# HengyiWang/MorpheuS

Hardware: AMD Instinct MI355X
Metric: rays/sec (fwd+bwd, 128 samples/ray) (higher is better)
Workload: dtype f32 (exact 3 x bf16 operand split on the bf16 MFMA pipe, fp32 accumulate)

## Files before the change

### morpheus_amd/csrc/mlp_b3.hip

```cpp
#include "mlp_dev.h"
#include <stdlib.h>

#define B3_THREADS 512
#define B3_BLOCK_PTS 256
#define B3_L0_F4 2560
#define B3_LH_F4 6144
#define B3_KH_F4 3072
#define B3_L5_F4 1536
#define B3_NET_F4 (B3_L0_F4 + 4 * B3_LH_F4 + B3_L5_F4)
#define B3_LDS_BYTES (B3_LH_F4 * 16 + 1024)

extern __shared__ f32x4 lds_b3[];
constexpr int B3_Q4_FILL = 6;
#define B3_PARK_STORES_EIGHTH 8
#define B3_PARK_STORES_HALF (4 * B3_PARK_STORES_EIGHTH)
#define B3_KEEP_BWD B3_PARK_STORES_HALF
static_assert(B3_KEEP_BWD <= B3_PARK_STORES_HALF && B3_PARK_STORES_HALF <= 63, "vmcnt(KEEP) must not exceed the stores behind the DMA");

#ifdef MH_PHASE_TRACE
__device__ long long mh_b3_trace[256 * 64];
#define B3_TRACE_ON (((threadIdx.x & 255) == 0) && (blockIdx.x % 64 == 0) && (blockIdx.x / 64 < 128))
#define B3_TRACE_ROW ((blockIdx.x / 64) * 2 + (threadIdx.x >> 8))
#define B3_STAMP(slot)                                                                          \
    do {                                                                                        \
        if (B3_TRACE_ON) mh_b3_trace[B3_TRACE_ROW * 64 + (slot)] = (long long)__builtin_amdgcn_s_memtime(); \
    } while (0)
#define B3_STAMP_REAL(slot)                                                                     \
    do {                                                                                        \
        if (B3_TRACE_ON) mh_b3_trace[B3_TRACE_ROW * 64 + (slot)] = (long long)__builtin_amdgcn_s_memrealtime(); \
    } while (0)
extern "C" int mh_b3_trace_read(long long *dst_host) {
    return hipMemcpyFromSymbol(dst_host, HIP_SYMBOL(mh_b3_trace), sizeof(long long) * 256 * 64) == hipSuccess ? 0 : 2;
}
#else
#define B3_STAMP(slot) do { } while (0)
#define B3_STAMP_REAL(slot) do { } while (0)
#endif

template <int N_F4, int NTHR = B3_THREADS>
__device__ __forceinline__ void b3_stage_issue(const f32x4 *__restrict__ src) {
    static_assert(N_F4 % NTHR == 0, "whole rounds of the block");
    const int wave = threadIdx.x >> 6;
#pragma unroll
    for (int k = 0; k < N_F4 / NTHR; k++)
        __builtin_amdgcn_global_load_lds((const __attribute__((address_space(1))) void *)(src + k * NTHR + threadIdx.x),
                                         (__attribute__((address_space(3))) void *)(lds_b3 + k * NTHR + wave * 64), 16, 0, 0);
}
__device__ __forceinline__ void b3_stage_wait() {
    asm volatile("s_waitcnt vmcnt(0)" ::: "memory");
    __syncthreads();
}
template <int YOUNGER>
__device__ __forceinline__ void b3_stage_wait_keep() {
    static_assert(YOUNGER >= 0 && YOUNGER <= 63, "vmcnt is a 6-bit field");
    asm volatile("s_waitcnt vmcnt(%0)" ::"n"(YOUNGER) : "memory");
    __syncthreads();
}
__device__ __forceinline__ void b3_dma_fence() { asm volatile("" ::: "memory"); }

template <int KS, int MT, bool ZERO = false>
__device__ __forceinline__ void b3_layer(const f32x4 *__restrict__ w, const Frag (&bh)[8], const Frag (&bm)[8], const Frag (&bl)[8],
                                         f32x16 (&acc)[MT], int lane) {
    constexpr int PL = MT * KS * 64;
    constexpr int NT = MT >= 2 ? 2 : 1;
    const f32x16 zero = {0.f, 0.f, 0.f, 0.f, 0.f, 0.f, 0.f, 0.f, 0.f, 0.f, 0.f, 0.f, 0.f, 0.f, 0.f, 0.f};
#pragma unroll
    for (int s = 0; s < KS; s++) {
#pragma unroll
        for (int mp = 0; mp < MT; mp += NT) {
            Frag ah[NT], am[NT], al[NT];
#pragma unroll
            for (int t = 0; t < NT; t++) {
                ah[t].f = w[0 * PL + ((mp + t) * KS + s) * 64 + lane];
                am[t].f = w[1 * PL + ((mp + t) * KS + s) * 64 + lane];
                al[t].f = w[2 * PL + ((mp + t) * KS + s) * 64 + lane];
            }
#pragma unroll
            for (int t = 0; t < NT; t++)
                acc[mp + t] = __builtin_amdgcn_mfma_f32_32x32x16_bf16(al[t].h, bh[s].h, (ZERO && s == 0) ? zero : acc[mp + t], 0, 0, 0);
#pragma unroll
            for (int t = 0; t < NT; t++) acc[mp + t] = __builtin_amdgcn_mfma_f32_32x32x16_bf16(am[t].h, bm[s].h, acc[mp + t], 0, 0, 0);
#pragma unroll
            for (int t = 0; t < NT; t++) acc[mp + t] = __builtin_amdgcn_mfma_f32_32x32x16_bf16(ah[t].h, bl[s].h, acc[mp + t], 0, 0, 0);
#pragma unroll
            for (int t = 0; t < NT; t++) acc[mp + t] = __builtin_amdgcn_mfma_f32_32x32x16_bf16(am[t].h, bh[s].h, acc[mp + t], 0, 0, 0);
#pragma unroll
            for (int t = 0; t < NT; t++) acc[mp + t] = __builtin_amdgcn_mfma_f32_32x32x16_bf16(ah[t].h, bm[s].h, acc[mp + t], 0, 0, 0);
#pragma unroll
            for (int t = 0; t < NT; t++) acc[mp + t] = __builtin_amdgcn_mfma_f32_32x32x16_bf16(ah[t].h, bh[s].h, acc[mp + t], 0, 0, 0);
        }
    }
}

__device__ __forceinline__ void mfma_results_settle() {
    __builtin_amdgcn_sched_barrier(0);
    asm volatile("s_nop 15");
    __builtin_amdgcn_sched_barrier(0);
}

template <int T0, int S0>
__device__ __forceinline__ void b3_quarter(const f32x4 *__restrict__ w, const Frag (&bh)[8], const Frag (&bm)[8], const Frag (&bl)[8],
                                           f32x16 (&acc)[4], int lane) {
    constexpr int PLH = 4 * 4 * 64;
#pragma unroll
    for (int s = S0; s < S0 + 4; s++) {
        Frag ah[2], am[2], al[2];
        const f32x4 *wk = w + (S0 / 4) * B3_KH_F4 + ((s & 3)) * 64 + lane;
#pragma unroll
        for (int t = 0; t < 2; t++) {
            ah[t].f = wk[0 * PLH + (T0 + t) * 256];
            am[t].f = wk[1 * PLH + (T0 + t) * 256];
            al[t].f = wk[2 * PLH + (T0 + t) * 256];
        }
#pragma unroll
        for (int t = 0; t < 2; t++) acc[T0 + t] = __builtin_amdgcn_mfma_f32_32x32x16_bf16(al[t].h, bh[s].h, acc[T0 + t], 0, 0, 0);
#pragma unroll
        for (int t = 0; t < 2; t++) acc[T0 + t] = __builtin_amdgcn_mfma_f32_32x32x16_bf16(am[t].h, bm[s].h, acc[T0 + t], 0, 0, 0);
#pragma unroll
        for (int t = 0; t < 2; t++) acc[T0 + t] = __builtin_amdgcn_mfma_f32_32x32x16_bf16(ah[t].h, bl[s].h, acc[T0 + t], 0, 0, 0);
#pragma unroll
        for (int t = 0; t < 2; t++) acc[T0 + t] = __builtin_amdgcn_mfma_f32_32x32x16_bf16(am[t].h, bh[s].h, acc[T0 + t], 0, 0, 0);
#pragma unroll
        for (int t = 0; t < 2; t++) acc[T0 + t] = __builtin_amdgcn_mfma_f32_32x32x16_bf16(ah[t].h, bm[s].h, acc[T0 + t], 0, 0, 0);
#pragma unroll
        for (int t = 0; t < 2; t++) acc[T0 + t] = __builtin_amdgcn_mfma_f32_32x32x16_bf16(ah[t].h, bh[s].h, acc[T0 + t], 0, 0, 0);
    }
}

template <int T0>
__device__ __forceinline__ void b3_quarter_step(const f32x4 *__restrict__ w, const Frag (&bh)[8], const Frag (&bm)[8],
                                                const Frag (&bl)[8], f32x16 (&acc)[4], int lane, int s) {
    constexpr int PLH = 4 * 4 * 64;
    Frag ah[2], am[2], al[2];
    const f32x4 *wk = w + (s >> 2) * B3_KH_F4 + (s & 3) * 64 + lane;
#pragma unroll
    for (int t = 0; t < 2; t++) {
        ah[t].f = wk[0 * PLH + (T0 + t) * 256];
        am[t].f = wk[1 * PLH + (T0 + t) * 256];
        al[t].f = wk[2 * PLH + (T0 + t) * 256];
    }
#pragma unroll
    for (int t = 0; t < 2; t++) acc[T0 + t] = __builtin_amdgcn_mfma_f32_32x32x16_bf16(al[t].h, bh[s].h, acc[T0 + t], 0, 0, 0);
#pragma unroll
    for (int t = 0; t < 2; t++) acc[T0 + t] = __builtin_amdgcn_mfma_f32_32x32x16_bf16(am[t].h, bm[s].h, acc[T0 + t], 0, 0, 0);
#pragma unroll
    for (int t = 0; t < 2; t++) acc[T0 + t] = __builtin_amdgcn_mfma_f32_32x32x16_bf16(ah[t].h, bl[s].h, acc[T0 + t], 0, 0, 0);
#pragma unroll
    for (int t = 0; t < 2; t++) acc[T0 + t] = __builtin_amdgcn_mfma_f32_32x32x16_bf16(am[t].h, bh[s].h, acc[T0 + t], 0, 0, 0);
#pragma unroll
    for (int t = 0; t < 2; t++) acc[T0 + t] = __builtin_amdgcn_mfma_f32_32x32x16_bf16(ah[t].h, bm[s].h, acc[T0 + t], 0, 0, 0);
#pragma unroll
    for (int t = 0; t < 2; t++) acc[T0 + t] = __builtin_amdgcn_mfma_f32_32x32x16_bf16(ah[t].h, bh[s].h, acc[T0 + t], 0, 0, 0);
}

template <bool PARK>
__device__ __forceinline__ void b3_epilogue_eighth(f32x16 (&acc)[4], float *__restrict__ ht, uint32_t (&mt)[4], int pt, int h,
                                                   Frag (&bh)[8], Frag (&bm)[8], Frag (&bl)[8], int t, int s2) {
#pragma unroll
    for (int r = 8 * s2; r < 8 * s2 + 8; r++) acc[t][r] = relu_i(acc[t][r]);
    if (PARK) {
#pragma unroll
        for (int r = 8 * s2; r < 8 * s2 + B3_PARK_STORES_EIGHTH; r++) PARK_STORE(acc[t][r], &ht[(32 * t + acc_row(r, h)) * TILE + pt]);
    }
    uint32_t m = 0;
#pragma unroll
    for (int r = 8 * s2 + 7; r >= 8 * s2; r--) m = push_nz(m, acc[t][r]);
    mt[t] |= m << (8 * s2);
#pragma unroll
    for (int e2 = 0; e2 < 4; e2++)
        split2(acc[t][8 * s2 + 2 * e2], acc[t][8 * s2 + 2 * e2 + 1], bh[2 * t + s2].u[e2], bm[2 * t + s2].u[e2], bl[2 * t + s2].u[e2]);
}

template <int T0, bool PARK>
__device__ __forceinline__ void b3_epilogue_half(f32x16 (&acc)[4], float *__restrict__ ht, uint32_t (&mt)[4], int pt, int h,
                                                 Frag (&bh)[8], Frag (&bm)[8], Frag (&bl)[8]) {
#pragma unroll
    for (int t = T0; t < T0 + 2; t++) {
#pragma unroll
        for (int r = 0; r < 16; r++) acc[t][r] = relu_i(acc[t][r]);
        if (PARK) {
#pragma unroll
            for (int r = 0; r < 16; r++) PARK_STORE(acc[t][r], &ht[(32 * t + acc_row(r, h)) * TILE + pt]);
        }
        uint32_t m = 0;
#pragma unroll
        for (int r = 15; r >= 0; r--) m = push_nz(m, acc[t][r]);
        mt[t] = m;
#pragma unroll
        for (int s2 = 0; s2 < 2; s2++)
#pragma unroll
            for (int e2 = 0; e2 < 4; e2++)
                split2(acc[t][8 * s2 + 2 * e2], acc[t][8 * s2 + 2 * e2 + 1], bh[2 * t + s2].u[e2], bm[2 * t + s2].u[e2],
                       bl[2 * t + s2].u[e2]);
    }
}

#define B3_SLOT_F4 B3_KH_F4
#define B3_BIASROW_F4 (2 * B3_SLOT_F4)
constexpr int B3_Q_FILL = 6;

template <int N_F4, int NTHR>
__device__ __forceinline__ void b3_slot_issue(const f32x4 *__restrict__ base, int off_f4, int slot) {
    static_assert(N_F4 % NTHR == 0, "whole rounds of the block");
    asm volatile("" : "+s"(off_f4));
    const f32x4 *src = base + off_f4 + threadIdx.x;
    f32x4 *dst = lds_b3 + slot * B3_SLOT_F4 + (threadIdx.x >> 6) * 64;
#pragma unroll
    for (int k = 0; k < N_F4 / NTHR; k++)
        __builtin_amdgcn_global_load_lds((const __attribute__((address_space(1))) void *)(src + k * NTHR),
                                         (__attribute__((address_space(3))) void *)(dst + k * NTHR), 16, 0, 0);
}
__device__ __forceinline__ void b3_bias_issue(const float *__restrict__ bias, int off_floats, int n_f4, int row) {
    asm volatile("" : "+s"(off_floats));
    if ((int)threadIdx.x < n_f4)
        __builtin_amdgcn_global_load_lds((const __attribute__((address_space(1))) void *)(reinterpret_cast<const f32x4 *>(bias + off_floats) + threadIdx.x),
                                         (__attribute__((address_space(3))) void *)(lds_b3 + B3_BIASROW_F4 + row * 32), 16, 0, 0);
}
template <int T0, int NT, int MT>
__device__ __forceinline__ void b3_acc_bias_row(f32x16 (&acc)[MT], int h, int row) {
    const f32x4 *b = lds_b3 + B3_BIASROW_F4 + row * 32;
#pragma unroll
    for (int t = T0; t < T0 + NT; t++)
#pragma unroll
        for (int r4 = 0; r4 < 4; r4++) {
            const f32x4 v = b[8 * t + 2 * r4 + h];
#pragma unroll
            for (int c = 0; c < 4; c++) acc[t][4 * r4 + c] = v[c];
        }
}
template <int KEEP>
__device__ __forceinline__ void b3_point() {
    static_assert(KEEP >= 0 && KEEP <= 63, "vmcnt is a 6-bit field");
    asm volatile("s_waitcnt vmcnt(%0) lgkmcnt(0)" ::"n"(KEEP) : "memory");
    __builtin_amdgcn_s_barrier();
    asm volatile("" ::: "memory");
}
template <int T0>
__device__ __forceinline__ void b3_step(const f32x4 *__restrict__ wk, const Frag (&bh)[8], const Frag (&bm)[8], const Frag (&bl)[8],
                                        f32x16 (&acc)[4], int lane, int s) {
    constexpr int PLH = 4 * 4 * 64;
    Frag ah[2], am[2], al[2];
    const f32x4 *w = wk + (s & 3) * 64 + lane;
#pragma unroll
    for (int t = 0; t < 2; t++) {
        ah[t].f = w[0 * PLH + (T0 + t) * 256];
        am[t].f = w[1 * PLH + (T0 + t) * 256];
        al[t].f = w[2 * PLH + (T0 + t) * 256];
    }
#pragma unroll
    for (int t = 0; t < 2; t++) acc[T0 + t] = __builtin_amdgcn_mfma_f32_32x32x16_bf16(al[t].h, bh[s].h, acc[T0 + t], 0, 0, 0);
#pragma unroll
    for (int t = 0; t < 2; t++) acc[T0 + t] = __builtin_amdgcn_mfma_f32_32x32x16_bf16(am[t].h, bm[s].h, acc[T0 + t], 0, 0, 0);
#pragma unroll
    for (int t = 0; t < 2; t++) acc[T0 + t] = __builtin_amdgcn_mfma_f32_32x32x16_bf16(ah[t].h, bl[s].h, acc[T0 + t], 0, 0, 0);
#pragma unroll
    for (int t = 0; t < 2; t++) acc[T0 + t] = __builtin_amdgcn_mfma_f32_32x32x16_bf16(am[t].h, bh[s].h, acc[T0 + t], 0, 0, 0);
#pragma unroll
    for (int t = 0; t < 2; t++) acc[T0 + t] = __builtin_amdgcn_mfma_f32_32x32x16_bf16(ah[t].h, bm[s].h, acc[T0 + t], 0, 0, 0);
#pragma unroll
    for (int t = 0; t < 2; t++) acc[T0 + t] = __builtin_amdgcn_mfma_f32_32x32x16_bf16(ah[t].h, bh[s].h, acc[T0 + t], 0, 0, 0);
}
__device__ __forceinline__ void b3_l5_step(const f32x4 *__restrict__ w, const Frag (&bh)[8], const Frag (&bm)[8], const Frag (&bl)[8],
                                           f32x16 &o, int lane, int s) {
    Frag ah, am, al;
    ah.f = w[0 * 512 + s * 64 + lane];
    am.f = w[1 * 512 + s * 64 + lane];
    al.f = w[2 * 512 + s * 64 + lane];
    o = __builtin_amdgcn_mfma_f32_32x32x16_bf16(al.h, bh[s].h, o, 0, 0, 0);
    o = __builtin_amdgcn_mfma_f32_32x32x16_bf16(am.h, bm[s].h, o, 0, 0, 0);
    o = __builtin_amdgcn_mfma_f32_32x32x16_bf16(ah.h, bl[s].h, o, 0, 0, 0);
    o = __builtin_amdgcn_mfma_f32_32x32x16_bf16(am.h, bh[s].h, o, 0, 0, 0);
    o = __builtin_amdgcn_mfma_f32_32x32x16_bf16(ah.h, bm[s].h, o, 0, 0, 0);
    o = __builtin_amdgcn_mfma_f32_32x32x16_bf16(ah.h, bh[s].h, o, 0, 0, 0);
}
template <int S0>
__device__ __forceinline__ void b3_pin_slices(Frag (&bh)[8], Frag (&bm)[8], Frag (&bl)[8]) {
#pragma unroll
    for (int s = S0; s < S0 + 4; s++)
        asm volatile("" : "+v"(bh[s].u[0]), "+v"(bh[s].u[1]), "+v"(bh[s].u[2]), "+v"(bh[s].u[3]), "+v"(bm[s].u[0]), "+v"(bm[s].u[1]),
                     "+v"(bm[s].u[2]), "+v"(bm[s].u[3]), "+v"(bl[s].u[0]), "+v"(bl[s].u[1]), "+v"(bl[s].u[2]), "+v"(bl[s].u[3]));
}
template <int N, int FILL>
__device__ __forceinline__ void b3_interleave() {
#pragma unroll
    for (int g = 0; g < N; g++) {
        __builtin_amdgcn_sched_group_barrier(0x008, 1, 0);
        __builtin_amdgcn_sched_group_barrier(0x002, FILL, 0);
    }
}

__device__ __forceinline__ uint32_t b3_or_half(uint32_t v) {
    v |= (uint32_t)__builtin_amdgcn_update_dpp(0, (int)v, 0x111, 0xf, 0xf, false);
    v |= (uint32_t)__builtin_amdgcn_update_dpp(0, (int)v, 0x112, 0xf, 0xf, false);
    v |= (uint32_t)__builtin_amdgcn_update_dpp(0, (int)v, 0x114, 0xf, 0xf, false);
    v |= (uint32_t)__builtin_amdgcn_update_dpp(0, (int)v, 0x118, 0xf, 0xf, false);
    v |= (uint32_t)__builtin_amdgcn_update_dpp(0, (int)v, 0x142, 0xa, 0xf, false);
    return v;
}
__device__ __forceinline__ void b3_park_line_word(float *__restrict__ tile, int idx, int pt, int h, uint32_t lo, uint32_t hi) {
    lo = b3_or_half(lo);
    hi = b3_or_half(hi);
    if (pt == 31) reinterpret_cast<uint2 *>(tile + WARP_LINE_ROW * TILE)[idx * 2 + h] = make_uint2(lo, hi);
}

template <int NW, bool PARK>
// ... 30 lines not shown

    for (int net = 0; net < 2; net++) {
        const f32x4 *wn = net ? w3_t : w3_d;
        const float *bs = net ? bias_t : bias_d;
        const float *b0 = (net ? bias0_t : bias0_d) + (int64_t)sl * 128;
        float *ht = PARK ? tile + (64 + net * 640) * TILE : nullptr;
        f32x16 acc[4];
        Frag bh[8], bm[8], bl[8];
        uint32_t mt[4] = {0u, 0u, 0u, 0u};
#pragma unroll
        for (int s = 0; s < 3; s++)
#pragma unroll
            for (int e2 = 0; e2 < 4; e2++) split2(bin0[8 * s + 2 * e2], bin0[8 * s + 2 * e2 + 1], bh[s].u[e2], bm[s].u[e2], bl[s].u[e2]);
        acc_bias<4>(acc, b0, h);
        b3_point<0>();
        b3_layer<3, 4>(slot0, bh, bm, bl, acc, lane);
        b3_point<0>();
        b3_slot_issue<B3_KH_F4, NT>(wn, B3_L0_F4 + B3_KH_F4, 0);
        b3_dma_fence();
        b3_epilogue_half<0, PARK>(acc, ht, mt, pt, h, bh, bm, bl);
        __builtin_amdgcn_sched_barrier(0);
        for (int l = 1; l <= 4; l++) {
            const int row = l & 1;
            float *hp = ht + (l - 1) * 128 * TILE, *hl = ht + l * 128 * TILE;
            if (net == 0) B3_STAMP((l - 1) * 8 + 0);
            if (net == 0 && l == 1) B3_STAMP_REAL(62);
            b3_acc_bias_row<0, 2, 4>(acc, h, row);
            mt[2] = mt[3] = 0u;
#pragma unroll
            for (int c = 0; c < 4; c++) {
                b3_step<0>(slot1, bh, bm, bl, acc, lane, c);
                b3_epilogue_eighth<PARK>(acc, hp, mt, pt, h, bh, bm, bl, 2 + (c >> 1), c & 1);
            }
            b3_pin_slices<4>(bh, bm, bl);
            asm volatile("" : "+v"(mt[2]), "+v"(mt[3]));
            b3_interleave<48, B3_Q_FILL>();
            __builtin_amdgcn_sched_barrier(0);
            if (PARK) {
                mk[(net * 5 + l - 1) * 64 + lane] = make_uint2(mt[0] | (mt[1] << 16), mt[2] | (mt[3] << 16));
                b3_park_line_word(tile, net * 5 + l - 1, pt, h, mt[0] | (mt[1] << 16), mt[2] | (mt[3] << 16));
            }
            if (net == 0) B3_STAMP((l - 1) * 8 + 1);
            b3_acc_bias_row<2, 2, 4>(acc, h, row);
#pragma unroll
            for (int c = 0; c < 4; c++) b3_step<2>(slot1, bh, bm, bl, acc, lane, c);
            __builtin_amdgcn_sched_barrier(0);
            if (net == 0) B3_STAMP((l - 1) * 8 + 2);
            b3_point<KEEP>();
            if (l < 4)
                b3_slot_issue<B3_KH_F4, NT>(wn, B3_L0_F4 + 2 * l * B3_KH_F4, 1);
            else
                b3_slot_issue<B3_L5_F4, NT>(wn, B3_L0_F4 + 8 * B3_KH_F4, 1);
            b3_bias_issue(bs, l * 128, l < 4 ? 32 : 8, (l + 1) & 1);
            b3_dma_fence();
            if (net == 0) B3_STAMP((l - 1) * 8 + 3);
#pragma unroll
            for (int c = 4; c < 8; c++) b3_step<0>(slot0, bh, bm, bl, acc, lane, c);
            __builtin_amdgcn_sched_barrier(0);
            if (net == 0) B3_STAMP((l - 1) * 8 + 4);
            mt[0] = mt[1] = 0u;
#pragma unroll
            for (int c = 0; c < 4; c++) {
                b3_step<2>(slot0, bh, bm, bl, acc, lane, 4 + c);
                b3_epilogue_eighth<PARK>(acc, hl, mt, pt, h, bh, bm, bl, c >> 1, c & 1);
            }
            b3_pin_slices<0>(bh, bm, bl);
            asm volatile("" : "+v"(mt[0]), "+v"(mt[1]));
            b3_interleave<48, B3_Q_FILL>();
            __builtin_amdgcn_sched_barrier(0);
            if (net == 0) B3_STAMP((l - 1) * 8 + 5);
            b3_point<KEEP>();
            if (l < 4)
                b3_slot_issue<B3_KH_F4, NT>(wn, B3_L0_F4 + (2 * l + 1) * B3_KH_F4, 0);
            else if (net == 0)
                b3_slot_issue<B3_L0_F4, NT>(w3_t, 0, 0);
            b3_dma_fence();
            if (net == 0) B3_STAMP((l - 1) * 8 + 6);
            if (net == 0 && l == 4) B3_STAMP_REAL(63);
        }
        f32x16 o[1];
        b3_acc_bias_row<0, 1, 1>(o, h, 1);
        mt[2] = mt[3] = 0u;
#pragma unroll
        for (int c = 0; c < 4; c++) {
            b3_l5_step(slot1, bh, bm, bl, o[0], lane, c);
            b3_epilogue_eighth<PARK>(acc, ht + 4 * 128 * TILE, mt, pt, h, bh, bm, bl, 2 + (c >> 1), c & 1);
        }
        b3_pin_slices<4>(bh, bm, bl);
        asm volatile("" : "+v"(mt[2]), "+v"(mt[3]));
        b3_interleave<24, 12>();
        __builtin_amdgcn_sched_barrier(0);
        if (PARK) {
            mk[(net * 5 + 4) * 64 + lane] = make_uint2(mt[0] | (mt[1] << 16), mt[2] | (mt[3] << 16));
            b3_park_line_word(tile, net * 5 + 4, pt, h, mt[0] | (mt[1] << 16), mt[2] | (mt[3] << 16));
        }
#pragma unroll
        for (int s = 4; s < 8; s++) b3_l5_step(slot1, bh, bm, bl, o[0], lane, s);
        b3_point<0>();
        if (net == 0) {
            b3_slot_issue<B3_KH_F4, NT>(w3_t, B3_L0_F4, 1);
            b3_bias_issue(bias_t, 0, 32, 1);
        }
        if (h == 0 && p < M && tile_raw < n_tiles) {
            if (net == 0) {
                out_deform[p * 3 + 0] = o[0][0];
                out_deform[p * 3 + 1] = o[0][1];
                out_deform[p * 3 + 2] = o[0][2];
            } else {
                out_topo[p * 2 + 0] = o[0][0];
                out_topo[p * 2 + 1] = o[0][1];
            }
        }
    }
}

#define B3_T5_F4 1536
#define B3_T0_F4 3072
#define B3_NETT_F4 (B3_T5_F4 + 4 * B3_LH_F4 + B3_T0_F4)

template <bool PARK = true>
__device__ __forceinline__ void b3_epilogue_bwd(const f32x16 (&acc)[4], uint2 m, float *__restrict__ dt, int pt, int h, Frag (&bh)[8],
                                                Frag (&bm)[8], Frag (&bl)[8]) {
    mfma_results_settle();
#pragma unroll
    for (int t = 0; t < 4; t++) {
        const uint32_t mw = (t < 2 ? m.x : m.y) >> (16 * (t & 1));
        float y[16];
#pragma unroll
        for (int r = 0; r < 16; r++) y[r] = mask_bit(mw, r, acc[t][r]);
        if (PARK) {
#pragma unroll
            for (int r = 0; r < 16; r++) PARK_STORE(y[r], &dt[(32 * t + acc_row(r, h)) * TILE + pt]);
        }
#pragma unroll
        for (int s2 = 0; s2 < 2; s2++)
#pragma unroll
            for (int e2 = 0; e2 < 4; e2++)
                split2(y[8 * s2 + 2 * e2], y[8 * s2 + 2 * e2 + 1], bh[2 * t + s2].u[e2], bm[2 * t + s2].u[e2], bl[2 * t + s2].u[e2]);
    }
}

__device__ __forceinline__ void b3_epilogue_bwd_eighth(f32x16 (&acc)[4], uint2 m, float *__restrict__ dt, int pt, int h, Frag (&bh)[8],
                                                       Frag (&bm)[8], Frag (&bl)[8], int t, int s2) {
    const uint32_t mw = (t < 2 ? m.x : m.y) >> (16 * (t & 1));
#pragma unroll
    for (int r = 8 * s2; r < 8 * s2 + 8; r++) acc[t][r] = mask_bit(mw, r, acc[t][r]);
#pragma unroll
    for (int r = 8 * s2; r < 8 * s2 + B3_PARK_STORES_EIGHTH; r++) PARK_STORE(acc[t][r], &dt[(32 * t + acc_row(r, h)) * TILE + pt]);
#pragma unroll
    for (int e2 = 0; e2 < 4; e2++)
        split2(acc[t][8 * s2 + 2 * e2], acc[t][8 * s2 + 2 * e2 + 1], bh[2 * t + s2].u[e2], bm[2 * t + s2].u[e2], bl[2 * t + s2].u[e2]);
}

template <int NW, bool PARK4 = true>
__global__ __launch_bounds__(NW * 64, 2) void warp_bwd_b3_kernel(const float *__restrict__ x, const float *__restrict__ g_deform,
                                                                 const float *__restrict__ g_topo, const f32x4 *__restrict__ w3T_d,
                                                                 const f32x4 *__restrict__ w3T_t, int n_bands,
                                                                 const float *__restrict__ acts, float *__restrict__ dpre,
                                                                 float *__restrict__ g_x, int64_t M, int64_t n_tiles) {
    const int lane = threadIdx.x & 63, wave = threadIdx.x >> 6;
    const int pt = lane & 31, h = lane >> 5;
    const int64_t tile_raw = (int64_t)blockIdx.x * NW + wave;
    const bool have = tile_raw < n_tiles;
    const int64_t tile_id = have ? tile_raw : n_tiles - 1;
    const int64_t p = tile_id * TILE + pt;
    const bool live = p < M;
    const float *atile = acts + tile_id * (int64_t)(WARP_ACT_ROWS * TILE);
    float *dtile = dpre + tile_id * (int64_t)(WARP_DPRE_ROWS * TILE);
    float gx[3] = {0.f, 0.f, 0.f};

    b3_stage_issue<B3_T5_F4, NW * 64>(w3T_d);
    for (int net = 0; net < 2; net++) {
        const f32x4 *wt = net ? w3T_t : w3T_d;
        const float *g = net ? g_topo : g_deform;
        const int nout = net ? 2 : 3;
        float *dt = dtile + net * 672 * TILE;
        const uint2 *mk = reinterpret_cast<const uint2 *>(atile + WARP_HID_ROWS * TILE) + net * 5 * 64 + lane;
        uint2 msk[5];
#pragma unroll
        for (int l = 0; l < 5; l++) msk[l] = mk[l * 64];
        float d5[16];
#pragma unroll
        for (int r = 0; r < 16; r++) d5[r] = 0.f;
        if (g && live && h == 0) {
            d5[0] = g[p * nout + 0];
            d5[1] = g[p * nout + 1];
            if (nout == 3) d5[2] = g[p * nout + 2];
        }
        if (h == 0) {
#pragma unroll
            for (int r = 0; r < 4; r++) dt[(640 + r) * TILE + pt] = d5[r];
        }
        Frag bh[8], bm[8], bl[8];
#pragma unroll
        for (int s = 0; s < 2; s++)
#pragma unroll
            for (int e2 = 0; e2 < 4; e2++) split2(d5[8 * s + 2 * e2], d5[8 * s + 2 * e2 + 1], bh[s].u[e2], bm[s].u[e2], bl[s].u[e2]);
        f32x16 acc[4];
        b3_stage_wait();
        b3_layer<2, 4, true>(lds_b3, bh, bm, bl, acc, lane);
        __syncthreads();
        wt += B3_T5_F4;
        b3_stage_issue<B3_LH_F4, NW * 64>(wt);
        b3_dma_fence();
        b3_epilogue_bwd<PARK4>(acc, msk[4], dt + 4 * 128 * TILE, pt, h, bh, bm, bl);
        for (int l = 4; l >= 1; l--) {
            if (!PARK4 && l == 4)
                b3_stage_wait();
            else
                b3_stage_wait_keep<B3_KEEP_BWD>();
            acc_zero<4>(acc);
            b3_quarter<0, 0>(lds_b3, bh, bm, bl, acc, lane);
            b3_quarter<2, 0>(lds_b3, bh, bm, bl, acc, lane);
            b3_quarter<0, 4>(lds_b3, bh, bm, bl, acc, lane);
            __builtin_amdgcn_sched_barrier(0);
#pragma unroll
            for (int c = 0; c < 4; c++) {
                b3_quarter_step<2>(lds_b3, bh, bm, bl, acc, lane, 4 + c);
                b3_epilogue_bwd_eighth(acc, msk[l - 1], dt + (l - 1) * 128 * TILE, pt, h, bh, bm, bl, c >> 1, c & 1);
            }
            b3_pin_slices<0>(bh, bm, bl);
#pragma unroll
            for (int g_ = 0; g_ < 48; g_++) {
                __builtin_amdgcn_sched_group_barrier(0x008, 1, 0);
                __builtin_amdgcn_sched_group_barrier(0x002, B3_Q4_FILL, 0);
            }
            __builtin_amdgcn_sched_barrier(0);
            __syncthreads();
            wt += B3_LH_F4;
            if (l > 1)
                b3_stage_issue<B3_LH_F4, NW * 64>(wt);
            else if (g_x)
                b3_stage_issue<B3_T0_F4, NW * 64>(wt);
            else if (net == 0)
                b3_stage_issue<B3_T5_F4, NW * 64>(w3T_t);
            b3_dma_fence();
#pragma unroll
            for (int c = 0; c < 4; c++)
                b3_epilogue_bwd_eighth(acc, msk[l - 1], dt + (l - 1) * 128 * TILE, pt, h, bh, bm, bl, 2 + (c >> 1), c & 1);
        }
        if (g_x) {
            f32x16 e[2];
            b3_stage_wait_keep<B3_KEEP_BWD>();
            b3_layer<8, 2, true>(lds_b3, bh, bm, bl, e, lane);
            __syncthreads();
            if (net == 0) b3_stage_issue<B3_T5_F4, NW * 64>(w3T_t);
            mfma_results_settle();
            float dsc[18];
            enc_deriv_parked(atile, pt, h, dsc);
#pragma unroll
            for (int k = 0; k < 18; k++) {
                const float de = k < 16 ? e[0][k] : e[1][k - 16];
                gx[k % 3] += de * dsc[k];
            }
            if (h == 0) {
                gx[0] += e[1][2];
                gx[2] += e[1][3];
            } else {
                gx[1] += e[1][2];
            }
        }
    }
#pragma unroll
    for (int d = 0; d < 3; d++) gx[d] += __shfl_xor(gx[d], 32);
    if (g_x && live && have && h == 0) {
        g_x[p * 3 + 0] = gx[0];
        g_x[p * 3 + 1] = gx[1];
        g_x[p * 3 + 2] = gx[2];
    }
}

#define FB3_S0 0
#define FB3_S1 2048
#define FB3_S2 3584
#define FB3_C0 5120
#define FB3_C1 6656
#define FB3_C2 8192
#define FB3_F4 9216
#define FB3_THREADS 512

__device__ __forceinline__ float laplace_sigma_b3(float s, float beta) {
    return (1.0f / beta) * laplace_unit(s, beta);
}

__device__ __forceinline__ void fb3_epilogue(f32x16 (&acc)[2], float *__restrict__ ht, uint32_t *__restrict__ mk, int pt, int h,
                                             Frag (&bh)[8], Frag (&bm)[8], Frag (&bl)[8]) {
    uint32_t m = 0;
#pragma unroll
    for (int t = 1; t >= 0; t--) {
#pragma unroll
        for (int r = 15; r >= 0; r--) {
            acc[t][r] = relu_i(acc[t][r]);
            m = push_nz(m, acc[t][r]);
        }
    }
#pragma unroll
    for (int t = 0; t < 2; t++) {
        if (ht) {
#pragma unroll
            for (int r = 0; r < 16; r++) PARK_STORE(acc[t][r], &ht[(32 * t + acc_row(r, h)) * TILE + pt]);
        }
#pragma unroll
        for (int s2 = 0; s2 < 2; s2++)
#pragma unroll
            for (int e2 = 0; e2 < 4; e2++)
                split2(acc[t][8 * s2 + 2 * e2], acc[t][8 * s2 + 2 * e2 + 1], bh[2 * t + s2].u[e2], bm[2 * t + s2].u[e2],
                       bl[2 * t + s2].u[e2]);
    }
    if (mk) *mk = m;
}

__device__ __forceinline__ void fb3_epilogue_plain(f32x16 (&acc)[2], float *__restrict__ ht, uint32_t *__restrict__ mk, int pt, int h) {
    uint32_t m = 0;
#pragma unroll
    for (int t = 1; t >= 0; t--) {
#pragma unroll
        for (int r = 15; r >= 0; r--) {
            acc[t][r] = relu_i(acc[t][r]);
            m = push_nz(m, acc[t][r]);
        }
    }
    if (ht) {
#pragma unroll
        for (int t = 0; t < 2; t++)
#pragma unroll
            for (int r = 0; r < 16; r++) PARK_STORE(acc[t][r], &ht[(32 * t + acc_row(r, h)) * TILE + pt]);
    }
    if (mk) *mk = m;
}

__global__ __launch_bounds__(FB3_THREADS, 2) void field_fwd_b3_kernel(
    const float *__restrict__ xc, const float *__restrict__ feat_s, const float *__restrict__ feat_c, const float *__restrict__ topo,
    const f32x4 *__restrict__ w3, const float *__restrict__ bias, const float *__restrict__ beta_p, int n_bands, int with_color,
    float *__restrict__ sdf, float *__restrict__ sigma, float *__restrict__ albedo, float *__restrict__ acts, int64_t M,
    int64_t n_tiles) {
    const int lane = threadIdx.x & 63, wave = threadIdx.x >> 6;
    const int pt = lane & 31, h = lane >> 5;
    {
        const int n = with_color ? FB3_F4 : FB3_C0;
        for (int i = threadIdx.x; i < n; i += FB3_THREADS) lds_b3[i] = w3[i];
    }
    __syncthreads();
    float *wsdf = reinterpret_cast<float *>(lds_b3 + FB3_C0);
    if (!with_color) {
        if (threadIdx.x < 64) {
            const int hh = threadIdx.x >> 5, kk = threadIdx.x & 31, s = kk >> 3, e = kk & 7;
            float v[3];
#pragma unroll
            for (int pl = 0; pl < 3; pl++) {
                Frag f;
                f.f = lds_b3[FB3_S2 + 4 * 64 + pl * 512 + s * 64 + 32 * hh];
                const uint32_t w = f.u[e >> 1];
                v[pl] = __uint_as_float((e & 1) ? (w & 0xffff0000u) : (w << 16));
            }
            wsdf[hh * 32 + kk] = (v[0] + v[1]) + v[2];
        }
        __syncthreads();
    }
    for (int64_t tile_id = (int64_t)blockIdx.x * (FB3_THREADS / 64) + wave; tile_id < n_tiles;
         tile_id += (int64_t)gridDim.x * (FB3_THREADS / 64)) {
        const int64_t p = tile_id * TILE + pt;
        const bool live = p < M;
        const int64_t pc = live ? p : M - 1;
        float xv[3] = {xc[pc * 3 + 0], xc[pc * 3 + 1], xc[pc * 3 + 2]};
        float *tile = acts ? acts + tile_id * (int64_t)(FIELD_ACT_ROWS * TILE) : nullptr;
        uint32_t *mk = tile ? reinterpret_cast<uint32_t *>(tile + FIELD_HID_ROWS * TILE) + lane : nullptr;
        Frag bh[8], bm[8], bl[8];
        f32x16 acc[2];
        {
            float bin0[40];
            enc_bin(xv, h, n_bands, bin0);
            const f32x4 *fs = reinterpret_cast<const f32x4 *>(feat_s + pc * 32 + 16 * h);
#pragma unroll
            for (int q = 0; q < 4; q++) {
                const f32x4 v = fs[q];
#pragma unroll
                for (int c = 0; c < 4; c++) bin0[20 + 4 * q + c] = v[c];
            }
            bin0[36] = topo ? topo[pc * 2 + h] : 0.f;
            bin0[37] = bin0[38] = bin0[39] = 0.f;
            if (tile) {
#pragma unroll
                for (int k = 0; k < 40; k++) PARK_STORE(bin0[k], &tile[(2 * k + h) * TILE + pt]);
            }
#pragma unroll
            for (int s = 0; s < 5; s++)
#pragma unroll
                for (int e2 = 0; e2 < 4; e2++) split2(bin0[8 * s + 2 * e2], bin0[8 * s + 2 * e2 + 1], bh[s].u[e2], bm[s].u[e2], bl[s].u[e2]);
        }
        acc_bias<2>(acc, bias, h);
        b3_layer<5, 2>(lds_b3 + FB3_S0, bh, bm, bl, acc, lane);
        fb3_epilogue(acc, tile ? tile + 96 * TILE : nullptr, mk ? mk + 0 * 64 : nullptr, pt, h, bh, bm, bl);
// ... 225 lines not shown
```

### morpheus_amd/packing.py

```python
from __future__ import annotations

from dataclasses import dataclass
from typing import Dict, List, Sequence, Tuple

import numpy as np
import torch


def acc_row(r: int, h: int) -> int:
    return (r & 3) + 8 * (r >> 2) + 4 * h


def kmap_acc(n_tiles: int) -> np.ndarray:
    km = np.zeros((16 * n_tiles, 2), dtype=np.int64)
    for kk in range(16 * n_tiles):
        t, r = kk >> 4, kk & 15
        for h in (0, 1):
            km[kk, h] = 32 * t + acc_row(r, h)
    return km


def kmap_enc20() -> np.ndarray:
    km = -np.ones((20, 2), dtype=np.int64)
    for kk in range(18):
        band, dim = kk // 3, kk % 3
        km[kk, 0] = 3 + band * 6 + dim
        km[kk, 1] = 3 + band * 6 + 3 + dim
    km[18] = (0, 1)
    km[19] = (2, -1)
    return km


def rowmapT_kk(kmap: np.ndarray, n_tiles: int) -> np.ndarray:
    rm = -np.ones(32 * n_tiles, dtype=np.int64)
    for rho in range(32 * n_tiles):
        t, q = rho >> 5, rho & 31
        h, r = (q >> 2) & 1, (q & 3) + 4 * (q >> 3)
        kk = 16 * t + r
        if kk < kmap.shape[0]:
            rm[rho] = kmap[kk, h]
    return rm


def _frag_index(row_of_lane: np.ndarray, col_of_k: np.ndarray, n_cols: int, transpose: bool, sentinel: int,
                base: int) -> np.ndarray:
    MT, KS = row_of_lane.shape[0] // 32, col_of_k.shape[0]
    idx = np.full((MT, KS // 4, 64, 4), sentinel, dtype=np.int64)
    for mt in range(MT):
        for kk in range(KS):
            q, j = kk // 4, kk % 4
            for lane in range(64):
                a = row_of_lane[mt * 32 + (lane & 31)]
                b = col_of_k[kk, lane >> 5]
                if a < 0 or b < 0:
                    continue
                idx[mt, q, lane, j] = base + ((b * n_cols + a) if transpose else (a * n_cols + b))
    return idx.reshape(-1)


def _frag_index_b3(row_of_lane: np.ndarray, col_of_k: np.ndarray, n_cols: int, transpose: bool, sentinel: int,
                   base: int) -> np.ndarray:
    MT, KS = row_of_lane.shape[0] // 32, col_of_k.shape[0]
    KS16 = (KS + 7) // 8
    km = np.full((KS16 * 8, 2), -1, dtype=np.int64)
    km[:KS] = col_of_k
    lane = np.arange(64)
    a = row_of_lane.reshape(MT, 32)[:, lane & 31]
    b = km.reshape(KS16, 8, 2)[:, :, lane >> 5].transpose(0, 2, 1)
    a4, b4 = a[:, None, :, None], b[None, :, :, :]
    flat = (b4 * n_cols + a4) if transpose else (a4 * n_cols + b4)
    idx = np.where((a4 >= 0) & (b4 >= 0), base + flat, sentinel)
    return idx.reshape(-1)


def _b3_blocks(idx: np.ndarray, MT: int, KS16: int):
    if MT == 4 and KS16 == 8:
        v = idx.reshape(4, 2, 4, 64, 8).transpose(1, 0, 2, 3, 4)
        return [v[0].reshape(-1), v[1].reshape(-1)]
    return [idx]


B3_DMA_F4 = 512


@dataclass
class LayerSpec:
    name: str
    out_dim: int
    in_dim: int
    kmap: np.ndarray
    rowmap: np.ndarray
    kmapT: np.ndarray
    rowmapT: np.ndarray
    act_rows: np.ndarray
    dpre_rows: np.ndarray


def _ident(n: int, pad: int) -> np.ndarray:
    v = -np.ones(pad, dtype=np.int64)
    v[:n] = np.arange(n)
    return v


def _kk_rows(kmap: np.ndarray, pad: int) -> np.ndarray:
    v = -np.ones(pad, dtype=np.int64)
    for kk in range(kmap.shape[0]):
        for h in (0, 1):
            v[2 * kk + h] = kmap[kk, h]
    return v


def warp_net_specs(n_out: int) -> List[LayerSpec]:
    enc = kmap_enc20()
    a128 = kmap_acc(4)
    a32 = kmap_acc(1)
    specs = [LayerSpec("l0", 128, 39, enc, _ident(128, 128), a128, rowmapT_kk(enc, 2), _kk_rows(enc, 64),
                       _ident(128, 128))]
    for l in range(1, 5):
        specs.append(LayerSpec(f"l{l}", 128, 128, a128, _ident(128, 128), a128, _ident(128, 128), _ident(128, 128),
                               _ident(128, 128)))
    kT = np.where(a32 < n_out, a32, -1)
    specs.append(LayerSpec("l5", n_out, 128, a128, _ident(n_out, 32), kT, _ident(128, 128), _ident(128, 128),
                           _ident(n_out, 32)))
    return specs


def field_specs() -> List[LayerSpec]:
    enc = kmap_enc20()
    a64 = kmap_acc(2)
    a32 = kmap_acc(1)
    k0 = -np.ones((40, 2), dtype=np.int64)
    k0[:20] = enc
    for kk in range(20, 36):
        k0[kk] = (39 + (kk - 20), 39 + 16 + (kk - 20))
    k0[36] = (71, 72)
    rT0 = -np.ones(96, dtype=np.int64)
    rT0[:64] = rowmapT_kk(enc, 2)
    for h in (0, 1):
        rT0[32 + acc_row(4, h)] = 71 + h
    for q in range(32):
        h, r = (q >> 2) & 1, (q & 3) + 4 * (q >> 3)
        rT0[64 + q] = 39 + 16 * h + r
    s0 = LayerSpec("s0", 64, 73, k0, _ident(64, 64), a64, rT0, _kk_rows(k0, 96), _ident(64, 64))
    s1 = LayerSpec("s1", 64, 64, a64, _ident(64, 64), a64, _ident(64, 64), _ident(64, 64), _ident(64, 64))
    r2 = -np.ones(64, dtype=np.int64)
    r2[:32] = 1 + np.arange(32)
    r2[32] = 0
    k2T = -np.ones((32, 2), dtype=np.int64)
    for kk in range(16):
        for h in (0, 1):
            k2T[kk, h] = 1 + acc_row(kk, h)
            k2T[16 + kk, h] = 0 if acc_row(kk, h) == 0 else -1
    s2 = LayerSpec("s2", 33, 64, a64, r2, k2T, _ident(64, 64), _ident(64, 64), r2.copy())
    kc = -np.ones((32, 2), dtype=np.int64)
    for kk in range(16):
        kc[kk] = (kk, 16 + kk)
        for h in (0, 1):
            kc[16 + kk, h] = 32 + acc_row(kk, h)
    rTc = -np.ones(64, dtype=np.int64)
    for q in range(32):
        h, r = (q >> 2) & 1, (q & 3) + 4 * (q >> 3)
        rTc[q] = 16 * h + r
        rTc[32 + q] = 32 + q
    c0 = LayerSpec("c0", 64, 64, kc, _ident(64, 64), a64, rTc, _kk_rows(kc, 64), _ident(64, 64))
    c1 = LayerSpec("c1", 64, 64, a64, _ident(64, 64), a64, _ident(64, 64), _ident(64, 64), _ident(64, 64))
    kT = np.where(a32 < 3, a32, -1)
    c2 = LayerSpec("c2", 3, 64, a64, _ident(3, 32), kT, _ident(64, 64), _ident(64, 64), _ident(3, 32))
    return [s0, s1, s2, c0, c1, c2]


class NetPacker:

    def __init__(self, specs: Sequence[LayerSpec], bwd_order: Sequence[int]):
        self.specs = list(specs)
        offs, n = [], 0
        for s in self.specs:
            offs.append(n)
            n += s.out_dim * s.in_dim
        self.w_offsets, self.n_weights = offs, n
        sentinel = n
        fwd = [_frag_index(s.rowmap, s.kmap, s.in_dim, False, sentinel, o) for s, o in zip(self.specs, offs)]
        bwd = [_frag_index(self.specs[i].rowmapT, self.specs[i].kmapT, self.specs[i].in_dim, True, sentinel, offs[i])
               for i in bwd_order]
        self.fwd_index = np.concatenate(fwd)
        self.bwd_index = np.concatenate(bwd)
        fwd3, self.fwd3_layer = [], []
        for li, (s, o) in enumerate(zip(self.specs, offs)):
            blocks = _b3_blocks(_frag_index_b3(s.rowmap, s.kmap, s.in_dim, False, sentinel, o), s.rowmap.shape[0] // 32,
                                (s.kmap.shape[0] + 7) // 8)
            fwd3 += blocks
            self.fwd3_layer += [li] * len(blocks)
        self.fwd3_index = np.concatenate(fwd3)
        self.fwd3_n = [len(f) for f in fwd3]
        self.fwd3_f4, f4 = [], 0
        for n in self.fwd3_n:
            self.fwd3_f4.append(f4)
            f4 += -(-(3 * n // 8) // B3_DMA_F4) * B3_DMA_F4
        self.fwd3_total_f4 = f4
        bwd3, self.bwd3_layer = [], []
        for li, i in enumerate(bwd_order):
            sp = self.specs[i]
            blocks = _b3_blocks(_frag_index_b3(sp.rowmapT, sp.kmapT, sp.in_dim, True, sentinel, offs[i]), sp.rowmapT.shape[0] // 32,
                                (sp.kmapT.shape[0] + 7) // 8)
            bwd3 += blocks
            self.bwd3_layer += [li] * len(blocks)
        self.bwd3_index = np.concatenate(bwd3)
        self.bwd3_n = [len(f) for f in bwd3]
        self.bwd3_f4, f4 = [], 0
        for n in self.bwd3_n:
            self.bwd3_f4.append(f4)
            f4 += -(-(3 * n // 8) // B3_DMA_F4) * B3_DMA_F4
        self.bwd3_total_f4 = f4
        b_offs, nb = [], 0
        for s in self.specs:
            b_offs.append(nb)
            nb += s.out_dim
        self.b_offsets, self.n_biases = b_offs, nb
        bidx = []
        for s, o in zip(self.specs, b_offs):
            bidx.append(np.where(s.rowmap >= 0, s.rowmap + o, nb))
        self.bias_index = bidx
        dw_idx, db_idx, raw_off, rawb_off = [], [], 0, 0
        self.wg_in, self.wg_out = [], []
        for s in self.specs:
            in_pad, out_pad = s.act_rows.shape[0], s.dpre_rows.shape[0]
            arow = -np.ones(s.in_dim, dtype=np.int64)
            for i, c in enumerate(s.act_rows):
                if c >= 0:
                    arow[c] = i
            drow = -np.ones(s.out_dim, dtype=np.int64)
            for i, r in enumerate(s.dpre_rows):
                if r >= 0:
                    drow[r] = i
            assert (arow >= 0).all() and (drow >= 0).all(), s.name
            dw_idx.append((raw_off + drow[:, None] * in_pad + arow[None, :]).reshape(-1))
            db_idx.append(rawb_off + drow)
            raw_off += in_pad * out_pad
            rawb_off += out_pad
            self.wg_in.append(in_pad)
            self.wg_out.append(out_pad)
        self.dw_index = np.concatenate(dw_idx)
        self.db_index = np.concatenate(db_idx)
        self.raw_dw, self.raw_db = raw_off, rawb_off
        self._dev: Dict[Tuple[str, int], Dict[str, torch.Tensor]] = {}

    def on(self, device: torch.device) -> Dict[str, torch.Tensor]:
        key = (device.type, device.index or 0)
        if key not in self._dev:
            t = lambda a: torch.from_numpy(np.ascontiguousarray(a)).to(device)
            self._dev[key] = dict(fwd=t(self.fwd_index), bwd=t(self.bwd_index), dw=t(self.dw_index), db=t(self.db_index),
                                  bias=[t(b) for b in self.bias_index])
        return self._dev[key]

    def flat_weights(self, weights: Sequence[torch.Tensor]) -> torch.Tensor:
        parts = [w.reshape(-1) for w in weights]
        return torch.cat(parts + [parts[0].new_zeros(1)])

    def pack(self, weights: Sequence[torch.Tensor]) -> Tuple[torch.Tensor, torch.Tensor]:
        m = self.on(weights[0].device)
        flat = self.flat_weights(weights)
        return flat[m["fwd"]].contiguous(), flat[m["bwd"]].contiguous()

    def pack_biases(self, biases: Sequence[torch.Tensor], skip_first: bool) -> torch.Tensor:
        m = self.on(biases[0].device)
        flat = torch.cat([b.reshape(-1) for b in biases] + [biases[0].new_zeros(1)])
        sel = m["bias"][1:] if skip_first else m["bias"]
        return torch.cat([flat[i] for i in sel]).contiguous()

    def unpack_grads(self, dw_raw: torch.Tensor, db_raw: torch.Tensor):
        m = self.on(dw_raw.device)
        dw = dw_raw[m["dw"]]
        db = db_raw[m["db"]]
        outw, outb, o, ob = [], [], 0, 0
        for s in self.specs:
            n = s.out_dim * s.in_dim
            outw.append(dw[o:o + n].view(s.out_dim, s.in_dim))
            outb.append(db[ob:ob + s.out_dim])
            o += n
            ob += s.out_dim
        return outw, outb


class JointPacker:

    def sliced_bwd_for(self, mode) -> bool:
        mode = "b3" if mode is True else mode
        return self.sliced_bwd and mode == "b3"

    def __init__(self, packers: Sequence[NetPacker], skip_first_bias: bool, sliced_bwd: bool = True):
        self.packers = list(packers)
        self.sliced_bwd = sliced_bwd
        nW = sum(p.n_weights for p in self.packers)
        nB = sum(p.n_biases for p in self.packers)
        zero = nW + nB
        fwd, bwd, bias = [], [], []
        self.w, self.wT, self.b = [], [], []
        wo, bo, f_off, t_off = 0, nW, 0, 0
        for p in self.packers:
            fwd.append(np.where(p.fwd_index == p.n_weights, zero, p.fwd_index + wo))
            bwd.append(np.where(p.bwd_index == p.n_weights, zero, p.bwd_index + wo))
            sel = p.bias_index[1:] if skip_first_bias else p.bias_index
            bi = np.concatenate(sel)
            bias.append(np.where(bi == p.n_biases, zero, bi + bo))
            self.w.append((f_off, len(p.fwd_index)))
            self.wT.append((t_off, len(p.bwd_index)))
            f_off += len(p.fwd_index)
            t_off += len(p.bwd_index)
            wo += p.n_weights
            bo += p.n_biases
        for bi in bias:
            self.b.append((f_off, len(bi)))
            f_off += len(bi)
        assert all(o % 4 == 0 for o, _ in self.w + self.wT + self.b), "kernel operands are read as float4"
        self.fwd_index = np.concatenate(fwd + bias)
        self.bwd_index = np.concatenate(bwd)
        self.n_flat = zero + 1
        f3, self.w3, self.b3_layers, wo, src, f4 = [], [], [], 0, 0, 0
        for p in self.packers:
            f3.append(np.where(p.fwd3_index == p.n_weights, zero, p.fwd3_index + wo))
            self.w3.append((f4, p.fwd3_total_f4))
            for n, o4 in zip(p.fwd3_n, p.fwd3_f4):
                self.b3_layers.append((src, n, f4 + o4))
                src += n
            f4 += p.fwd3_total_f4
            wo += p.n_weights
        self.fwd3_index = np.concatenate(f3)
        self.fwd3_total_f4 = f4
        t3, self.wT3, self.b3T_layers, wo, src, f4 = [], [], [], 0, 0, 0
        for p in self.packers:
            t3.append(np.where(p.bwd3_index == p.n_weights, zero, p.bwd3_index + wo))
            self.wT3.append((f4, p.bwd3_total_f4))
            for n, o4 in zip(p.bwd3_n, p.bwd3_f4):
                self.b3T_layers.append((src, n, f4 + o4))
                src += n
            f4 += p.bwd3_total_f4
            wo += p.n_weights
        self.bwd3_index = np.concatenate(t3)
        self.bwd3_total_f4 = f4
        raw_dw = sum(p.raw_dw for p in self.packers)
        g, dwo, dbo = [], 0, raw_dw
        for p in self.packers:
            g.append(p.dw_index + dwo)
            dwo += p.raw_dw
        for p in self.packers:
            g.append(p.db_index + dbo)
            dbo += p.raw_db
        self.grad_index = np.concatenate(g)
        self.raw_len = dbo
        self.bias0_raw, off = [], raw_dw
        for p in self.packers:
            self.bias0_raw.append(off)
            off += p.raw_db
        gz = self.grad_index.copy()
        pos = sum(p.n_weights for p in self.packers)
        for p in self.packers:
            gz[pos:pos + p.specs[0].out_dim] = self.raw_len
# ... 92 lines not shown
```

Baseline: 1.087 million.

## Switch backward hidden-layer MFMA from 32x32x16 to 16x16x32 with permlane repacking

The backward hidden-layer GEMM now uses 16x16x32 bf16 MFMA instead of 32x32x16. The host repacks the transposed weight fragments into a new layout, and the kernel uses permlane16 swaps to convert the activation slices into block form and to restore accumulator row order before each epilogue. The scheduling group pattern is retuned for twice as many, smaller MFMAs. The aim is a shorter MFMA issue latency and finer interleaving with LDS reads, at the cost of extra permlane instructions and more MFMA issues.

```diff
diff --git a/morpheus_amd/csrc/mlp_b3.hip b/morpheus_amd/csrc/mlp_b3.hip
--- a/morpheus_amd/csrc/mlp_b3.hip
+++ b/morpheus_amd/csrc/mlp_b3.hip
@@ -96,61 +96,6 @@
     __builtin_amdgcn_sched_barrier(0);
     asm volatile("s_nop 15");
     __builtin_amdgcn_sched_barrier(0);
-}
-
-template <int T0, int S0>
-__device__ __forceinline__ void b3_quarter(const f32x4 *__restrict__ w, const Frag (&bh)[8], const Frag (&bm)[8], const Frag (&bl)[8],
-                                           f32x16 (&acc)[4], int lane) {
-    constexpr int PLH = 4 * 4 * 64;
-#pragma unroll
-    for (int s = S0; s < S0 + 4; s++) {
-        Frag ah[2], am[2], al[2];
-        const f32x4 *wk = w + (S0 / 4) * B3_KH_F4 + ((s & 3)) * 64 + lane;
-#pragma unroll
-        for (int t = 0; t < 2; t++) {
-            ah[t].f = wk[0 * PLH + (T0 + t) * 256];
-            am[t].f = wk[1 * PLH + (T0 + t) * 256];
-            al[t].f = wk[2 * PLH + (T0 + t) * 256];
-        }
-#pragma unroll
-        for (int t = 0; t < 2; t++) acc[T0 + t] = __builtin_amdgcn_mfma_f32_32x32x16_bf16(al[t].h, bh[s].h, acc[T0 + t], 0, 0, 0);
-#pragma unroll
-        for (int t = 0; t < 2; t++) acc[T0 + t] = __builtin_amdgcn_mfma_f32_32x32x16_bf16(am[t].h, bm[s].h, acc[T0 + t], 0, 0, 0);
-#pragma unroll
-        for (int t = 0; t < 2; t++) acc[T0 + t] = __builtin_amdgcn_mfma_f32_32x32x16_bf16(ah[t].h, bl[s].h, acc[T0 + t], 0, 0, 0);
-#pragma unroll
-        for (int t = 0; t < 2; t++) acc[T0 + t] = __builtin_amdgcn_mfma_f32_32x32x16_bf16(am[t].h, bh[s].h, acc[T0 + t], 0, 0, 0);
-#pragma unroll
-        for (int t = 0; t < 2; t++) acc[T0 + t] = __builtin_amdgcn_mfma_f32_32x32x16_bf16(ah[t].h, bm[s].h, acc[T0 + t], 0, 0, 0);
-#pragma unroll
-        for (int t = 0; t < 2; t++) acc[T0 + t] = __builtin_amdgcn_mfma_f32_32x32x16_bf16(ah[t].h, bh[s].h, acc[T0 + t], 0, 0, 0);
-    }
-}
-
-template <int T0>
-__device__ __forceinline__ void b3_quarter_step(const f32x4 *__restrict__ w, const Frag (&bh)[8], const Frag (&bm)[8],
-                                                const Frag (&bl)[8], f32x16 (&acc)[4], int lane, int s) {
-    constexpr int PLH = 4 * 4 * 64;
-    Frag ah[2], am[2], al[2];
-    const f32x4 *wk = w + (s >> 2) * B3_KH_F4 + (s & 3) * 64 + lane;
-#pragma unroll
-    for (int t = 0; t < 2; t++) {
-        ah[t].f = wk[0 * PLH + (T0 + t) * 256];
-        am[t].f = wk[1 * PLH + (T0 + t) * 256];
-        al[t].f = wk[2 * PLH + (T0 + t) * 256];
-    }
-#pragma unroll
-    for (int t = 0; t < 2; t++) acc[T0 + t] = __builtin_amdgcn_mfma_f32_32x32x16_bf16(al[t].h, bh[s].h, acc[T0 + t], 0, 0, 0);
-#pragma unroll
-    for (int t = 0; t < 2; t++) acc[T0 + t] = __builtin_amdgcn_mfma_f32_32x32x16_bf16(am[t].h, bm[s].h, acc[T0 + t], 0, 0, 0);
-#pragma unroll
-    for (int t = 0; t < 2; t++) acc[T0 + t] = __builtin_amdgcn_mfma_f32_32x32x16_bf16(ah[t].h, bl[s].h, acc[T0 + t], 0, 0, 0);
-#pragma unroll
-    for (int t = 0; t < 2; t++) acc[T0 + t] = __builtin_amdgcn_mfma_f32_32x32x16_bf16(am[t].h, bh[s].h, acc[T0 + t], 0, 0, 0);
-#pragma unroll
-    for (int t = 0; t < 2; t++) acc[T0 + t] = __builtin_amdgcn_mfma_f32_32x32x16_bf16(ah[t].h, bm[s].h, acc[T0 + t], 0, 0, 0);
-#pragma unroll
-    for (int t = 0; t < 2; t++) acc[T0 + t] = __builtin_amdgcn_mfma_f32_32x32x16_bf16(ah[t].h, bh[s].h, acc[T0 + t], 0, 0, 0);
 }
 
 template <bool PARK>
@@ -487,6 +432,71 @@
         split2(acc[t][8 * s2 + 2 * e2], acc[t][8 * s2 + 2 * e2 + 1], bh[2 * t + s2].u[e2], bm[2 * t + s2].u[e2], bl[2 * t + s2].u[e2]);
 }
 
+__device__ __forceinline__ void b3n_swap(uint32_t &x, uint32_t &y) {
+    const auto s = __builtin_amdgcn_permlane16_swap(x, y, false, false);
+    x = s[0];
+    y = s[1];
+}
+template <int S0>
+__device__ __forceinline__ void b3n_slices_to_blocks(Frag (&bh)[8], Frag (&bm)[8], Frag (&bl)[8]) {
+#pragma unroll
+    for (int s = S0; s < S0 + 4; s += 2)
+#pragma unroll
+        for (int e = 0; e < 4; e++) {
+            b3n_swap(bh[s].u[e], bh[s + 1].u[e]);
+            b3n_swap(bm[s].u[e], bm[s + 1].u[e]);
+            b3n_swap(bl[s].u[e], bl[s + 1].u[e]);
+        }
+}
+__device__ __forceinline__ void b3n_acc_swap_eighth(f32x16 (&acc)[4], int t, int s2) {
+#pragma unroll
+    for (int r = 0; r < 4; r++) {
+        uint32_t x = __float_as_uint(acc[t][8 * s2 + r]), y = __float_as_uint(acc[t][8 * s2 + 4 + r]);
+        b3n_swap(x, y);
+        acc[t][8 * s2 + r] = __uint_as_float(x);
+        acc[t][8 * s2 + 4 + r] = __uint_as_float(y);
+    }
+}
+template <int T>
+__device__ __forceinline__ void b3n_tile_step(const f32x4 *__restrict__ w, const Frag (&bh)[8], const Frag (&bm)[8], const Frag (&bl)[8],
+                                              f32x16 (&acc)[4], int lane, int S) {
+    constexpr int PLH = 4 * 4 * 64;
+    Frag ah[2], am[2], al[2];
+    const f32x4 *wk = w + (S >> 1) * B3_KH_F4 + T * 256 + (S & 1) * 64 + lane;
+#pragma unroll
+    for (int u = 0; u < 2; u++) {
+        ah[u].f = wk[0 * PLH + u * 128];
+        am[u].f = wk[1 * PLH + u * 128];
+        al[u].f = wk[2 * PLH + u * 128];
+    }
+#define B3N_MM(A, B)                                                                                                   \
+    _Pragma("unroll") for (int u = 0; u < 2; u++) _Pragma("unroll") for (int b = 0; b < 2; b++) {                      \
+        const int q = 8 * u + 4 * b;                                                                                   \
+        f32x4 c = {acc[T][q], acc[T][q + 1], acc[T][q + 2], acc[T][q + 3]};                                            \
+        c = __builtin_amdgcn_mfma_f32_16x16x32_bf16(A[u].h, B[2 * S + b].h, c, 0, 0, 0);                               \
+        acc[T][q] = c[0];                                                                                              \
+        acc[T][q + 1] = c[1];                                                                                          \
+        acc[T][q + 2] = c[2];                                                                                          \
+        acc[T][q + 3] = c[3];                                                                                          \
+    }
+    B3N_MM(al, bh)
+    B3N_MM(am, bm)
+    B3N_MM(ah, bl)
+    B3N_MM(am, bh)
+    B3N_MM(ah, bm)
+    B3N_MM(ah, bh)
+#undef B3N_MM
+}
+template <int T0, int S0>
+__device__ __forceinline__ void b3n_quarter(const f32x4 *__restrict__ w, const Frag (&bh)[8], const Frag (&bm)[8], const Frag (&bl)[8],
+                                            f32x16 (&acc)[4], int lane) {
+#pragma unroll
+    for (int S = S0; S < S0 + 2; S++) {
+        b3n_tile_step<T0>(w, bh, bm, bl, acc, lane, S);
+        b3n_tile_step<T0 + 1>(w, bh, bm, bl, acc, lane, S);
+    }
+}
+
 template <int NW, bool PARK4 = true>
 __global__ __launch_bounds__(NW * 64, 2) void warp_bwd_b3_kernel(const float *__restrict__ x, const float *__restrict__ g_deform,
                                                                  const float *__restrict__ g_topo, const f32x4 *__restrict__ w3T_d,
@@ -545,20 +555,26 @@
             else
                 b3_stage_wait_keep<B3_KEEP_BWD>();
             acc_zero<4>(acc);
-            b3_quarter<0, 0>(lds_b3, bh, bm, bl, acc, lane);
-            b3_quarter<2, 0>(lds_b3, bh, bm, bl, acc, lane);
-            b3_quarter<0, 4>(lds_b3, bh, bm, bl, acc, lane);
+            b3n_slices_to_blocks<0>(bh, bm, bl);
+            b3n_slices_to_blocks<4>(bh, bm, bl);
+            b3n_quarter<0, 0>(lds_b3, bh, bm, bl, acc, lane);
+            b3n_quarter<2, 0>(lds_b3, bh, bm, bl, acc, lane);
+            b3n_quarter<0, 2>(lds_b3, bh, bm, bl, acc, lane);
             __builtin_amdgcn_sched_barrier(0);
 #pragma unroll
             for (int c = 0; c < 4; c++) {
-                b3_quarter_step<2>(lds_b3, bh, bm, bl, acc, lane, 4 + c);
+                if (c & 1)
+                    b3n_tile_step<3>(lds_b3, bh, bm, bl, acc, lane, 2 + (c >> 1));
+                else
+                    b3n_tile_step<2>(lds_b3, bh, bm, bl, acc, lane, 2 + (c >> 1));
+                b3n_acc_swap_eighth(acc, c >> 1, c & 1);
                 b3_epilogue_bwd_eighth(acc, msk[l - 1], dt + (l - 1) * 128 * TILE, pt, h, bh, bm, bl, c >> 1, c & 1);
             }
             b3_pin_slices<0>(bh, bm, bl);
 #pragma unroll
-            for (int g_ = 0; g_ < 48; g_++) {
+            for (int g_ = 0; g_ < 96; g_++) {
                 __builtin_amdgcn_sched_group_barrier(0x008, 1, 0);
-                __builtin_amdgcn_sched_group_barrier(0x002, B3_Q4_FILL, 0);
+                __builtin_amdgcn_sched_group_barrier(0x002, B3_Q4_FILL / 2, 0);
             }
             __builtin_amdgcn_sched_barrier(0);
             __syncthreads();
@@ -571,8 +587,10 @@
                 b3_stage_issue<B3_T5_F4, NW * 64>(w3T_t);
             b3_dma_fence();
 #pragma unroll
-            for (int c = 0; c < 4; c++)
+            for (int c = 0; c < 4; c++) {
+                b3n_acc_swap_eighth(acc, 2 + (c >> 1), c & 1);
                 b3_epilogue_bwd_eighth(acc, msk[l - 1], dt + (l - 1) * 128 * TILE, pt, h, bh, bm, bl, 2 + (c >> 1), c & 1);
+            }
         }
         if (g_x) {
             f32x16 e[2];
diff --git a/morpheus_amd/packing.py b/morpheus_amd/packing.py
--- a/morpheus_amd/packing.py
+++ b/morpheus_amd/packing.py
@@ -78,6 +78,20 @@
         v = idx.reshape(4, 2, 4, 64, 8).transpose(1, 0, 2, 3, 4)
         return [v[0].reshape(-1), v[1].reshape(-1)]
     return [idx]
+
+
+def _b3_blocks_n16(idx: np.ndarray):
+    old = idx.reshape(4, 8, 64, 8)
+    new = np.empty((2, 4, 4, 64, 8), dtype=idx.dtype)
+    lane = np.arange(64)
+    j, g = lane & 15, lane >> 4
+    for kh in range(2):
+        for u in range(2):
+            for s1 in range(2):
+                S = 2 * kh + s1
+                row = 16 * u + 8 * ((j >> 2) & 1) + 4 * (j >> 3) + (j & 3)
+                new[kh, :, 2 * u + s1] = old[:, 2 * S + (g & 1), row + 32 * (g >> 1)]
+    return [new[0].reshape(-1), new[1].reshape(-1)]
 
 
 B3_DMA_F4 = 512
@@ -200,8 +214,9 @@
         bwd3, self.bwd3_layer = [], []
         for li, i in enumerate(bwd_order):
             sp = self.specs[i]
-            blocks = _b3_blocks(_frag_index_b3(sp.rowmapT, sp.kmapT, sp.in_dim, True, sentinel, offs[i]), sp.rowmapT.shape[0] // 32,
-                                (sp.kmapT.shape[0] + 7) // 8)
+            idx3 = _frag_index_b3(sp.rowmapT, sp.kmapT, sp.in_dim, True, sentinel, offs[i])
+            MT3, KS3 = sp.rowmapT.shape[0] // 32, (sp.kmapT.shape[0] + 7) // 8
+            blocks = _b3_blocks_n16(idx3) if (MT3 == 4 and KS3 == 8) else _b3_blocks(idx3, MT3, KS3)
             bwd3 += blocks
             self.bwd3_layer += [li] * len(blocks)
         self.bwd3_index = np.concatenate(bwd3)
```

Result: no change. 1.092 million (median of 6 runs) (+0.5%).
